# clancylian/retinaface

Hardware: NVIDIA B200
Metric: faces/sec (end-to-end detect) (higher is better)
Workload: dtype f16

## Files before the change

### retinaface_b200/csrc/engine_internal.cuh

```cuda
#pragma once
#include <algorithm>
#include <cstdarg>
#include <cstdio>
#include <cstring>
#include <functional>
#include <map>
#include <memory>
#include <string>
#include <type_traits>
#include <vector>

#include "common.cuh"
#include "host_copy.h"
#include "model.h"
#include "postproc.cuh"
#include "preprocess.cuh"

using namespace rf;

#define RF_STR2(x) #x
#define RF_STR(x) RF_STR2(x)

namespace rf_eng {

struct TileChain;
std::string &create_error();

struct CudaFail { cudaError_t e; const char *what; const char *file; int line; };
struct PlanFail { int status; std::string msg; };
#define CK(call)                                                        \
    do {                                                                \
        cudaError_t _e = (call);                                        \
        if (_e != cudaSuccess) throw CudaFail{_e, #call, __FILE__, __LINE__}; \
    } while (0)

inline std::string fmt(const char *f, ...) {
    char buf[1024];
    va_list ap;
    va_start(ap, f);
    vsnprintf(buf, sizeof buf, f, ap);
    va_end(ap);
    return buf;
}
// ... 179 lines not shown
        size_t off = h->wstage_q.size();
        h->wstage_q.insert(h->wstage_q.end(), v.begin(), v.end());
        while (h->wstage_q.size() % 128) h->wstage_q.push_back(0);
        return off;
    }
    int tensor(const std::string &name, int hh, int ww, int c) {
        TensorInfo t;
        t.name = name; t.h = hh; t.w = ww; t.c = c;
        t.bytes_per_img = (size_t)hh * ww * c * h->elem;
        h->tensors.push_back(t);
        h->tensor_by_name[name] = (int)h->tensors.size() - 1;
        return (int)h->tensors.size() - 1;
    }
    void step(Step s) { h->steps.push_back(std::move(s)); }
};

constexpr int TC_SMEM_LIMIT = 200 * 1024;
struct DwGeom { int rows, nsplit, Rmax; };
template <typename T>
void build_plan(rf_handle h);
cudaError_t tc_init();
std::vector<__half> make_stem_blob(const std::vector<float> &w0, const std::vector<float> &b0, const std::vector<float> &wd,
                                   const std::vector<float> &bd, const std::vector<float> &wp, const std::vector<float> &bp);
int plan_stem_tc(Builder &B);
int plan_pair_legacy(Builder &B, int i, int tin, int ih, int iw);
void plan_conv_legacy(Builder &B, const std::string &sname, std::vector<const FoldedConv *> cs, int tin, int ih, int iw, int t0, int ld0,
                      int off0, int n0, int relu0, int t1, int ld1, int off1, int relu1, int lane = 0, int tup = -1, int up_which = 0);
int plan_fpn_merge_h2(Builder &B, const std::string &name, int tlat, int tup, int fh, int fw, int which);
template <typename T>
void plan_heads_and_nms(Builder &B, bool with_heads, bool with_nms);
std::vector<__half> pack_tc_weights(const std::vector<const FoldedConv *> &cs, std::vector<float> &bias, int &Kpad, int nsplit = 1);
void build_plan_tiles(rf_handle h);
cudaError_t tile_init();
std::string describe_chains(rf_handle h);
void comm_release(rf_handle h);
void comm_wait_in_graph(rf_handle h, int n, cudaStream_t s);
int jpeg_info(rf_handle h, const uint8_t *data, size_t len, int *w, int *hgt);
int jpeg_decode(rf_handle h, const uint8_t *const *data, const size_t *len, int n, uint8_t *const *dst, const int *w, const int *hgt, cudaStream_t s);
void jpeg_release(rf_handle h);
const char *jpeg_backend(rf_handle h);
void build_plan_i8(rf_handle h);
cudaError_t tc_init_i8();

}
```

### retinaface_b200/csrc/plan_fp.cu

```cuda
#include "engine_internal.cuh"
#include "kernels_simt.cuh"
#include "stem_tc.cuh"
#include "tc_conv.cuh"
#include "tc_dwpw2d.cuh"

namespace rf_eng {

#define CK_L(...) CK(launch_k(__VA_ARGS__))

std::vector<float> pack_gemm(const std::vector<const FoldedConv *> &cs, std::vector<float> &bias) {
    const int cin = cs[0]->cin, k = cs[0]->k;
    int N = 0;
    for (auto c : cs) N += c->cout;
    std::vector<float> w((size_t)k * k * cin * N);
    bias.assign(N, 0.f);
    int n0 = 0;
    for (auto c : cs) {
        for (int o = 0; o < c->cout; o++) {
            bias[n0 + o] = c->b[o];
            for (int ci = 0; ci < cin; ci++)
                for (int t = 0; t < k * k; t++)
                    w[((size_t)t * cin + ci) * N + n0 + o] = c->w[((size_t)o * cin + ci) * k * k + t];
        }
        n0 += c->cout;
// ... 56 lines not shown
    TcDwArgs a = a_in;
    a.mul_Wp = fast_div_mul((uint32_t)a.Wp); a.mul_Hp = fast_div_mul((uint32_t)a.Hp);
    a.mul_OW = fast_div_mul((uint32_t)a.OW); a.mul_OH = fast_div_mul((uint32_t)a.OH);
    const long M = (long)a.nimg * a.OH * a.OW;
    dim3 grid((unsigned)((M + a.rows - 1) / a.rows), nsplit);
    const size_t smem = tc_dw_smem_bytes(a);
    switch (tc_tmem_cols(a.N)) {
        case 32: if (a.C >= 64) CK_L(k_tc_dwpw_staged<32, true>, grid, dim3(TC_THREADS), smem, s, a); else CK_L(k_tc_dwpw_staged<32, false>, grid, dim3(TC_THREADS), smem, s, a); break;
        case 64: if (a.C >= 64) CK_L(k_tc_dwpw_staged<64, true>, grid, dim3(TC_THREADS), smem, s, a); else CK_L(k_tc_dwpw_staged<64, false>, grid, dim3(TC_THREADS), smem, s, a); break;
        case 128: if (a.C >= 64) CK_L(k_tc_dwpw_staged<128, true>, grid, dim3(TC_THREADS), smem, s, a); else CK_L(k_tc_dwpw_staged<128, false>, grid, dim3(TC_THREADS), smem, s, a); break;
        default: if (a.C >= 64) CK_L(k_tc_dwpw_staged<256, true>, grid, dim3(TC_THREADS), smem, s, a); else CK_L(k_tc_dwpw_staged<256, false>, grid, dim3(TC_THREADS), smem, s, a); break;
    }
}
void launch_tc_dwpw_2d(const TcDw2dArgs &a, cudaStream_t s) {
    const dim3 grid((unsigned)(a.tiles_x * a.tiles_y * a.nimg));
    const size_t smem = tc_dw2d_smem_bytes(a);
    switch (tc_tmem_cols(a.N)) {
        case 32: CK_L(k_tc_dwpw_2d<32>, grid, dim3(TC_THREADS), smem, s, a); break;
        case 64: CK_L(k_tc_dwpw_2d<64>, grid, dim3(TC_THREADS), smem, s, a); break;
        case 128: CK_L(k_tc_dwpw_2d<128>, grid, dim3(TC_THREADS), smem, s, a); break;
        default: CK_L(k_tc_dwpw_2d<256>, grid, dim3(TC_THREADS), smem, s, a); break;
    }
}

cudaError_t tc_init() {
    cudaError_t e;
#define RF_TC_ATTR(K_) if ((e = cudaFuncSetAttribute(K_, cudaFuncAttributeMaxDynamicSharedMemorySize, TC_SMEM_LIMIT))) return e
    RF_TC_ATTR((k_tc_conv_staged<32, false>)); RF_TC_ATTR((k_tc_conv_staged<64, false>)); RF_TC_ATTR((k_tc_conv_staged<128, false>)); RF_TC_ATTR((k_tc_conv_staged<256, false>));
    RF_TC_ATTR((k_tc_conv_staged<32, true>)); RF_TC_ATTR((k_tc_conv_staged<64, true>)); RF_TC_ATTR((k_tc_conv_staged<128, true>)); RF_TC_ATTR((k_tc_conv_staged<256, true>));
    RF_TC_ATTR((k_tc_dwpw_staged<32, true>)); RF_TC_ATTR((k_tc_dwpw_staged<64, true>)); RF_TC_ATTR((k_tc_dwpw_staged<128, true>)); RF_TC_ATTR((k_tc_dwpw_staged<256, true>));
    RF_TC_ATTR((k_tc_dwpw_staged<32, false>)); RF_TC_ATTR((k_tc_dwpw_staged<64, false>)); RF_TC_ATTR((k_tc_dwpw_staged<128, false>)); RF_TC_ATTR((k_tc_dwpw_staged<256, false>));
    RF_TC_ATTR(k_tc_dwpw_2d<32>); RF_TC_ATTR(k_tc_dwpw_2d<64>); RF_TC_ATTR(k_tc_dwpw_2d<128>); RF_TC_ATTR(k_tc_dwpw_2d<256>);
#undef RF_TC_ATTR
    return cudaSuccess;
}

DwGeom dw_geometry(int C, int N, int IH, int IW, int S) {
    const int OH = IH / S, OW = IW / S, Wp = IW + 2, Hp = IH + 1, Kpad = (C + 15) / 16 * 16;
    auto centre = [&](long m) { long ox = m % OW, oy = (m / OW) % OH, b = m / ((long)OW * OH); return (b * Hp + oy * S) * Wp + ox * S + 1; };
    for (int rows : {128, 64}) {
        if (rows == 128 && OH * OW <= 28 * 28) continue;
        for (int nsplit : {1, 2, 4}) {
            if ((N / nsplit) % 16) continue;
            long g = rows, t = (long)OH * OW;
            while (t) { long u = g % t; g = t; t = u; }
            const long M = ((long)rows / g + 1) * OH * OW;
            int R = 0;
            for (long m0 = 0; m0 < M; m0 += rows) {
                long ml = std::min(m0 + rows, M) - 1;
                R = std::max(R, (int)(centre(ml) - centre(m0) + 2 * (Wp + 1) + 1));
            }
            R |= 1;
            TcDwArgs a{};
            a.C = C; a.Rmax = R; a.Kpad = Kpad; a.N = N / nsplit; a.rows = rows;
            if (R <= TC_MAX_R && tc_dw_smem_bytes(a) <= (size_t)TC_SMEM_LIMIT) return {rows, nsplit, R};
        }
    }
    return {0, 0, 0};
}

std::vector<__half> make_stem_blob(const std::vector<float> &w0, const std::vector<float> &b0, const std::vector<float> &wd,
                                          const std::vector<float> &bd, const std::vector<float> &wp, const std::vector<float> &bp) {
    std::vector<__half> b0img(2 * 4 * 16 * 8, __float2half(0.f)), b1img(2 * 16 * 8, __float2half(0.f));
    for (int k = 0; k < 27; k++)
        for (int o = 0; o < 8; o++) {
            const float wv = w0[k * 8 + o];
            const __half hi = __float2half(wv);
            b0img[((k / 8) * 16 + o) * 8 + (k % 8)] = hi;
            b0img[((4 + k / 8) * 16 + o) * 8 + (k % 8)] = __float2half(wv - __half2float(hi));
        }
    for (int c = 0; c < 8; c++)
        for (int o = 0; o < 16; o++) b1img[(0 * 16 + o) * 8 + c] = __float2half(wp[c * 16 + o]);
    std::vector<__half> blob(STEM_CONST_BYTES / 2, __float2half(0.f));
    memcpy(blob.data(), b0img.data(), STEM_B0_BYTES);
    memcpy(reinterpret_cast<unsigned char *>(blob.data()) + STEM_B0_BYTES, b1img.data(), STEM_B1_BYTES);
    std::vector<float> fl;
    fl.insert(fl.end(), b0.begin(), b0.begin() + 8);
    fl.insert(fl.end(), wd.begin(), wd.begin() + 72);
    fl.insert(fl.end(), bd.begin(), bd.begin() + 8);
    fl.insert(fl.end(), bp.begin(), bp.begin() + 16);
    fl.insert(fl.end(), wp.begin(), wp.begin() + 128);
    memcpy(reinterpret_cast<unsigned char *>(blob.data()) + STEM_B0_BYTES + STEM_B1_BYTES, fl.data(), STEM_F_FLOATS * 4);
    return blob;
}


int plan_pair_legacy(Builder &B, int i, int tin, int ih, int iw) {
    rf_handle h = B.h;
    const Model &m = h->model;
    auto T_ = [h](int id) { return reinterpret_cast<__half *>(h->tptr(id)); };
    auto Wd = [h](size_t off) { return h->d_weights + off; };
    const double es = h->elem;
    const FoldedConv &dw = m.conv("mobilenet0_conv" + std::to_string(i) + "_fwd");
    const FoldedConv &pw = m.conv("mobilenet0_conv" + std::to_string(i + 1) + "_fwd");
    const int C = dw.cout, S = dw.stride;
    std::vector<float> wd(9 * C);
    for (int c = 0; c < C; c++)
        for (int t = 0; t < 9; t++) wd[t * C + c] = dw.w[(size_t)c * 9 + t];
    size_t owd = B.add_weights(wd), obd = B.add_weights(dw.b);
    const int oh = ih / S, ow_ = iw / S;
    const int N = pw.cout;
    const DwGeom geo = dw_geometry(C, N, ih, iw, S);
    if (geo.rows == 0) throw PlanFail{RF_ERR_UNSUPPORTED, fmt("layer mobilenet0_conv%d (%dx%d, %d channels) does not fit shared memory", i, iw, ih, C)};
    std::vector<float> bias;
    int Kpad = 0;
    std::vector<__half> img = pack_tc_weights({&pw}, bias, Kpad, geo.nsplit);
    size_t oimg = B.add_weights_h(img), obp = B.add_weights(bias);
    int tpw = B.tensor("mobilenet0_relu" + std::to_string(i + 1) + "_fwd", oh, ow_, N);
    Step s;
    s.name = fmt("tc_dw%d+pw%d_s%d_%dto%d", i, i + 1, S, C, N);
    s.in = {tin}; s.out = {tpw};
    s.flops_per_img = 2.0 * oh * ow_ * C * 9 + 2.0 * oh * ow_ * C * N;
    s.bytes_per_img = ((double)ih * iw * C + (double)oh * ow_ * N) * es;
    const bool tiles2d = oh * ow_ > 56 * 56 && C >= 16 && C <= 64 && geo.nsplit == 1 && !(h->cfg.flags & RF_FLAG_DW_1D);
    if (tiles2d) s.name = fmt("tc2d_dw%d+pw%d_s%d_%dto%d", i, i + 1, S, C, N);
    s.launch = [=](int n, cudaStream_t st) {
        if (tiles2d) {
            TcDw2dArgs a{};
            a.in = T_(tin); a.C = C; a.nimg = n; a.IH = ih; a.IW = iw; a.OH = oh; a.OW = ow_; a.S = S; a.N = N;
            a.TH = 8;
            const int t16 = (ow_ + 15) / 16, t14 = (ow_ + 13) / 14;
            a.TW = t14 < t16 ? 14 : 16;
            tc_dw2d_finish(a);
            a.wimg = h->d_weights_h + oimg; a.bias = Wd(obp); a.dw_w = Wd(owd); a.dw_b = Wd(obd); a.out = T_(tpw);
            launch_tc_dwpw_2d(a, st);
            return;
        }
        TcDwArgs a{};
        a.in = T_(tin); a.C = C; a.nimg = n; a.IH = ih; a.IW = iw; a.OH = oh; a.OW = ow_; a.S = S;
        a.N = N / geo.nsplit; a.Ntotal = N; a.Kpad = Kpad; a.rows = geo.rows; a.Wp = iw + 2; a.Hp = ih + 1; a.Rmax = geo.Rmax;
        a.wimg = h->d_weights_h + oimg; a.bias = Wd(obp); a.dw_w = Wd(owd); a.dw_b = Wd(obd); a.out = T_(tpw);
        launch_tc_dwpw(a, geo.nsplit, st);
    };
    B.step(std::move(s));
    return tpw;
}

void plan_conv_legacy(Builder &B, const std::string &sname, std::vector<const FoldedConv *> cs, int tin, int ih, int iw, int t0, int ld0,
                      int off0, int n0, int relu0, int t1, int ld1, int off1, int relu1, int lane, int tup, int up_which) {
    rf_handle h = B.h;
    const Model &m = h->model;
    auto T_ = [h](int id) { return reinterpret_cast<__half *>(h->tptr(id)); };
    auto Wd = [h](size_t off) { return h->d_weights + off; };
    const double es = h->elem;
    std::vector<float> bias;
    int Kpad = 0;
    std::vector<__half> img = pack_tc_weights(cs, bias, Kpad);
    size_t oimg = B.add_weights_h(img), ob = B.add_weights(bias);
    const int N = (int)bias.size(), cin = cs[0]->cin, ks = cs[0]->k;
    size_t oup = tup >= 0 ? B.add_weights(m.up_w[up_which]) : 0;
    if (cin & (cin - 1)) throw PlanFail{RF_ERR_UNSUPPORTED, fmt("convolution %s: %d input channels (the tensor-core kernels index by shifts: powers of two only)", sname.c_str(), cin)};
    TcConvArgs probe{};
    probe.Cin = cin; probe.taps = ks * ks; probe.N = N; probe.R = (ks == 3 ? 128 + 2 * (iw + 3) : 128) | 1;
    if (tup >= 0) { probe.up = reinterpret_cast<const __half *>(1); probe.Cmax = (((probe.R / (iw + 2) + 2) / 2 + 3) * (iw / 2)) | 1; }
    if (tc_conv_smem_bytes(probe) > (size_t)TC_SMEM_LIMIT || probe.R > TC_MAX_R)
        throw PlanFail{RF_ERR_UNSUPPORTED, fmt("convolution %s (%dx%d map) does not fit shared memory", sname.c_str(), iw, ih)};
    Step s;
// ... 353 lines not shown
```

### retinaface_b200/csrc/plan_tile.cu

```cuda
#include <cstdlib>

#include "engine_internal.cuh"
#include "tile_chain.cuh"

namespace rf_eng {

namespace {

typedef CUresult (*EncodeTiledFn)(CUtensorMap *, CUtensorMapDataType, cuuint32_t, void *, const cuuint64_t *, const cuuint64_t *,
                                  const cuuint32_t *, const cuuint32_t *, CUtensorMapInterleave, CUtensorMapSwizzle, CUtensorMapL2promotion,
                                  CUtensorMapFloatOOBfill);
EncodeTiledFn g_encode = nullptr;

constexpr int TCH_SMEM_LIMIT = 226 * 1024;

CUtensorMap make_map(const void *base, int C, int W, int H, int n, int bc, int bw, int bh, int es) {
    CUtensorMap m;
    cuuint64_t dims[4] = {(cuuint64_t)C, (cuuint64_t)W, (cuuint64_t)H, (cuuint64_t)n};
    cuuint64_t strides[3] = {(cuuint64_t)C * 2, (cuuint64_t)W * C * 2, (cuuint64_t)H * W * C * 2};
    cuuint32_t box[4] = {(cuuint32_t)bc, (cuuint32_t)bw, (cuuint32_t)bh, 1};
    cuuint32_t est[4] = {1, (cuuint32_t)es, (cuuint32_t)es, 1};
    const CUtensorMapSwizzle sw = bc * 2 == 128 ? CU_TENSOR_MAP_SWIZZLE_128B : (bc * 2 == 64 ? CU_TENSOR_MAP_SWIZZLE_64B : CU_TENSOR_MAP_SWIZZLE_32B);
    CUresult r = g_encode(&m, CU_TENSOR_MAP_DATA_TYPE_FLOAT16, 4, const_cast<void *>(base), dims, strides, box, est, CU_TENSOR_MAP_INTERLEAVE_NONE, sw,
                          CU_TENSOR_MAP_L2_PROMOTION_L2_128B, CU_TENSOR_MAP_FLOAT_OOB_FILL_NONE);
    if (r != CUDA_SUCCESS) throw PlanFail{RF_ERR_CUDA, fmt("cuTensorMapEncodeTiled failed (%d) for a %dx%dx%d tensor, box %dx%dx%d", (int)r, C, W, H, bc, bw, bh)};
    return m;
}

int round_up(int v, int a) { return (v + a - 1) / a * a; }

}

struct TileChain {
    struct LBuf {
        int C = 0;
        int halo = 0;
        bool stored = false;
        int store_tensor = -1;
        int first = 1 << 30, last = -1;
        bool is_input = false, is_merge = false;
    };
    struct LStage {
        int type = TCH_CONV, Cin = 0, N = 0, taps = 1, stride = 1, in_buf = 0;
        std::vector<int> ob_buf, ob_c16, ob_relu;
        std::vector<__half> wd_img, wp_img;
        std::vector<float> bd, bp;
        int hs = 0;
        int store_buf = -1;
        double flops = 0;
    };
    std::string name;
    std::vector<LBuf> bufs;
    std::vector<LStage> stages;
    int in_tensor = -1, in_C = 0, in_W = 0, in_H = 0, in_s2 = 0;
    int W = 0, H = 0;
    int merge_tensor = -1;
    std::vector<__half> merge_w;
    int level = -1;
    bool fused_nms = false;
    TchArgs args{};
    size_t bias_off = 0;
    int store_buf_of[3] = {-1, -1, -1}, store_C[3] = {0, 0, 0};
    int nstores = 0;
// ... 333 lines not shown
void add_chain_step(Builder &B, std::shared_ptr<TileChain> c, int lane, double bytes_per_img) {
    rf_handle h = B.h;
    commit_chain(B, *c);
    h->chains.push_back(c);
    Step s;
    s.name = c->name;
    s.lane = lane;
    s.in = {c->in_tensor};
    if (c->merge_tensor >= 0) s.in.push_back(c->merge_tensor);
    for (int i = 0; i < c->nstores; i++) s.out.push_back(c->bufs[c->store_buf_of[i]].store_tensor);
    double fl = 0;
    for (auto &ls : c->stages) fl += ls.flops * c->W * c->H;
    s.flops_per_img = fl;
    s.bytes_per_img = bytes_per_img;
    s.launch = [h, c](int n, cudaStream_t st) { launch_chain(h, c, n, st); };
    B.step(std::move(s));
}

}

std::string describe_chains(rf_handle h) {
    std::string out;
    for (auto &cp : h->chains) {
        const TileChain &c = *cp;
        const TchArgs &a = c.args;
        out += fmt("%s: %dx%d map, TH=%d HT=%d Wl=%d, %d tiles/image, %d stages, %d MMA tiles/tile, smem %d B (%s weights), TMEM %d x %d cols, stores %d\n",
                   c.name.c_str(), c.W, c.H, a.TH, a.HT, a.Wl, a.tiles_per_img, a.nstages, c.mtiles, a.smem_bytes, a.resident ? "resident" : "streamed", a.nsets,
                   a.set_cols, c.nstores);
    }
    return out;
}

cudaError_t tile_init() {
    if (!g_encode) {
        void *fn = nullptr;
        cudaDriverEntryPointQueryResult q;
        cudaError_t e = cudaGetDriverEntryPoint("cuTensorMapEncodeTiled", &fn, cudaEnableDefault, &q);
        if (e != cudaSuccess) return e;
        if (!fn) return cudaErrorNotSupported;
        g_encode = (EncodeTiledFn)fn;
    }
    return cudaFuncSetAttribute(k_tile_chain<0>, cudaFuncAttributeMaxDynamicSharedMemorySize, TCH_SMEM_LIMIT);
}

enum { TM_A = 1, TM_B = 2, TM_C = 4, TM_D = 8, TM_E = 16, TM_AGGR = 32, TM_SSH = 64, TM_HEAD = 128, TM_NMS = 256, TM_ALL = 511 };
constexpr unsigned TM_LATENCY = TM_SSH | TM_HEAD | TM_NMS;
constexpr unsigned TM_LATENCY_SMALL = TM_AGGR | TM_SSH | TM_HEAD | TM_NMS;
constexpr unsigned TM_THROUGHPUT = 0;

static bool build_tiles_with_mask(rf_handle h, unsigned mask) {
    Builder B{h, h->cfg.net_h, h->cfg.net_w};
    const Model &m = h->model;
    const int H = h->cfg.net_h, W = h->cfg.net_w, mb = h->cfg.max_batch, mf = h->cfg.max_faces;
    if (!(mask & TM_SSH)) mask &= ~(TM_HEAD | TM_NMS);
    if (!(mask & TM_HEAD)) mask &= ~TM_NMS;
    const double es = 2;
    auto pair = [&](int i) -> std::pair<const FoldedConv *, const FoldedConv *> {
        return {&m.conv("mobilenet0_conv" + std::to_string(i) + "_fwd"), &m.conv("mobilenet0_conv" + std::to_string(i + 1) + "_fwd")};
    };
    auto relu_name = [](int i) { return "mobilenet0_relu" + std::to_string(i) + "_fwd"; };

    int cur = plan_stem_tc(B);
    int cur_h = H / 2, cur_w = W / 2, cur_c = 16;

    int lat1 = -1, lat2 = -1, lat3 = -1;
    auto backbone = [&](const std::string &name, std::vector<int> is, bool enabled, const char *lat_conv, int *lat_out, int lane_lat) {
        const int S = pair(is[0]).first->stride;
        const int oh = cur_h / S, ow = cur_w / S;
        const int Cout = pair(is.back()).second->cout;
        bool done = false;
        if (enabled) {
            auto c = std::make_shared<TileChain>();
            c->name = "tile_" + name;
            c->in_tensor = cur; c->in_C = cur_c; c->in_W = cur_w; c->in_H = cur_h; c->in_s2 = S == 2;
// ... 184 lines not shown
```

### retinaface_b200/csrc/tc_conv.cuh

```cuda
#pragma once
#include "common.cuh"

namespace rf {

constexpr int TC_LBO_A = 128 * 16 + 16;

struct TcOut {
    __half *p0; int ld0; int n0; int relu0;
    __half *p1; int ld1; int relu1;
};

namespace tc {

__device__ __forceinline__ uint32_t smem_u32(const void *p) { return (uint32_t)__cvta_generic_to_shared(p); }

__device__ __forceinline__ void mbar_init(uint64_t *bar, unsigned count) {
    asm volatile("mbarrier.init.shared::cta.b64 [%0], %1;" ::"r"(smem_u32(bar)), "r"(count));
}
__device__ __forceinline__ void mbar_expect_tx(uint64_t *bar, unsigned bytes) {
    asm volatile("mbarrier.arrive.expect_tx.shared::cta.b64 _, [%0], %1;" ::"r"(smem_u32(bar)), "r"(bytes) : "memory");
}
__device__ __forceinline__ void mbar_wait(uint64_t *bar, unsigned parity) {
    unsigned done = 0;
    unsigned spins = 0;
    while (!done) {
        asm volatile(
            "{\n\t.reg .pred p;\n\t"
            "mbarrier.try_wait.parity.shared::cta.b64 p, [%1], %2;\n\t"
            "selp.u32 %0, 1, 0, p;\n\t}"
            : "=r"(done)
            : "r"(smem_u32(bar)), "r"(parity)
            : "memory");
        if (!done && ++spins > (1u << 24)) __trap();
    }
}
__device__ __forceinline__ void bulk_g2s(void *dst, const void *src, unsigned bytes, uint64_t *bar) {
    asm volatile("cp.async.bulk.shared::cluster.global.mbarrier::complete_tx::bytes [%0], [%1], %2, [%3];" ::"r"(smem_u32(dst)),
                 "l"(src), "r"(bytes), "r"(smem_u32(bar))
                 : "memory");
}
__device__ __forceinline__ void fence_async_smem() { asm volatile("fence.proxy.async.shared::cta;" ::: "memory"); }
__device__ __forceinline__ void tc_fence_before() { asm volatile("tcgen05.fence::before_thread_sync;" ::: "memory"); }
__device__ __forceinline__ void tc_fence_after() { asm volatile("tcgen05.fence::after_thread_sync;" ::: "memory"); }

template <int COLS>
__device__ __forceinline__ void tmem_alloc(uint32_t *slot) {
    asm volatile("tcgen05.alloc.cta_group::1.sync.aligned.shared::cta.b32 [%0], %1;" ::"r"(smem_u32(slot)), "n"(COLS) : "memory");
    asm volatile("tcgen05.relinquish_alloc_permit.cta_group::1.sync.aligned;" ::: "memory");
}
template <int COLS>
__device__ __forceinline__ void tmem_dealloc(uint32_t addr) {
    asm volatile("tcgen05.dealloc.cta_group::1.sync.aligned.b32 %0, %1;" ::"r"(addr), "n"(COLS) : "memory");
}
__device__ __forceinline__ void mma_commit(uint64_t *bar) {
    asm volatile("tcgen05.commit.cta_group::1.mbarrier::arrive::one.shared::cluster.b64 [%0];" ::"r"(smem_u32(bar)) : "memory");
}
__device__ __forceinline__ void mma_f16(uint32_t d_tmem, uint64_t adesc, uint64_t bdesc, uint32_t idesc, uint32_t accumulate) {
    asm volatile(
        "{\n\t.reg .pred p;\n\t"
        "setp.ne.b32 p, %4, 0;\n\t"
        "tcgen05.mma.cta_group::1.kind::f16 [%0], %1, %2, %3, p;\n\t}"
        ::"r"(d_tmem), "l"(adesc), "l"(bdesc), "r"(idesc), "r"(accumulate)
        : "memory");
}
__device__ __forceinline__ uint64_t smem_desc(uint32_t addr, uint32_t lbo_bytes, uint32_t sbo_bytes) {
    uint64_t d = 0;
    d |= (uint64_t)((addr >> 4) & 0x3FFF);
    d |= (uint64_t)((lbo_bytes >> 4) & 0x3FFF) << 16;
    d |= (uint64_t)((sbo_bytes >> 4) & 0x3FFF) << 32;
    d |= (uint64_t)1 << 46;
    return d;
// ... 424 lines not shown
```

### retinaface_b200/csrc/tc_dwpw2d.cuh

```cuda
#pragma once
#include "tc_conv.cuh"

namespace rf {

struct TcDw2dArgs {
    const __half *in;
    int C, nimg, IH, IW, OH, OW, S;
    int N;
    int TH, TW;
    int tiles_x, tiles_y;
    int PH, PW;
    uint32_t lbo_a;
    uint32_t mul_TW, mul_tiles_x, mul_tiles;
    const __half *wimg;
    const float *bias;
    const float *dw_w, *dw_b;
    __half *out;
};

inline void tc_dw2d_finish(TcDw2dArgs &a) {
    const int G = a.C >> 3;
    a.PH = (a.TH - 1) * a.S + 3;
    a.PW = (a.TW - 1) * a.S + 3;
    a.tiles_x = (a.OW + a.TW - 1) / a.TW;
    a.tiles_y = (a.OH + a.TH - 1) / a.TH;
    a.lbo_a = (uint32_t)(128 + 8 / G) * 16;
    a.mul_TW = fast_div_mul((uint32_t)a.TW);
    a.mul_tiles_x = fast_div_mul((uint32_t)a.tiles_x);
    a.mul_tiles = fast_div_mul((uint32_t)(a.tiles_x * a.tiles_y));
}
inline size_t tc_dw2d_smem_bytes(const TcDw2dArgs &a) {
    return (size_t)a.PH * a.PW * a.C * 2 + (size_t)(a.C / 8) * a.lbo_a + (size_t)a.C * a.N * 2 + 128;
}

#ifndef RF_DW2D_OCC
#define RF_DW2D_OCC 6
#endif
template <int NT>
__global__ void __launch_bounds__(TC_THREADS, RF_DW2D_OCC) k_tc_dwpw_2d(const TcDw2dArgs a) {
    extern __shared__ __align__(128) unsigned char smem[];
    __shared__ __align__(8) uint64_t bar_b, bar_done;
    __shared__ uint32_t s_tmem;
    __shared__ float s_bias[256];
    __shared__ __align__(16) __half s_dwh[9 * 64];
    __shared__ __align__(16) float s_dwb[64];

    const int tid = threadIdx.x, warp = tid >> 5, lane = tid & 31;
    const int G = a.C >> 3, lg = 31 - __clz(G);
    const int PH = a.PH, PW = a.PW;
    const uint32_t lbo_a = a.lbo_a;
    const int pix = a.C * 2;
    unsigned char *sS = smem;
    unsigned char *sA = smem + (size_t)PH * PW * pix;
    unsigned char *sB = sA + (size_t)G * lbo_a;
    const int tiles = a.tiles_x * a.tiles_y;
    const int b = fast_div((int)blockIdx.x, a.mul_tiles), trem = blockIdx.x - b * tiles;
    const int ty0 = fast_div(trem, a.mul_tiles_x);
    const int oy0 = ty0 * a.TH, ox0 = (trem - ty0 * a.tiles_x) * a.TW;
    const int iy0 = oy0 * a.S - 1, ix0 = ox0 * a.S - 1;

    if (tid == 0) {
        tc::mbar_init(&bar_b, 1);
        tc::mbar_init(&bar_done, 1);
        asm volatile("fence.mbarrier_init.release.cluster;" ::: "memory");
        const unsigned bytes = (unsigned)((size_t)a.C * a.N * 2);
        tc::mbar_expect_tx(&bar_b, bytes);
        tc::bulk_g2s(sB, a.wimg, bytes, &bar_b);
    }
    if (warp == 1) tc::tmem_alloc<NT>(&s_tmem);
    pdl_trigger();
    if (tid < a.N) s_bias[tid] = a.bias[tid];
    for (int i = tid; i < 9 * a.C; i += TC_THREADS) s_dwh[i] = __float2half_rn(a.dw_w[i]);
    if (tid < a.C) s_dwb[tid] = a.dw_b[tid];
    pdl_wait();
    {
        const int per_row = PW << lg;
        const int px_lo = max(0, -ix0), px_hi = min(PW, a.IW - ix0);
        const unsigned px_n = (unsigned)max(px_hi - px_lo, 0);
        const uint32_t sS_s = tc::smem_u32(sS);
        for (int py = warp; py < PH; py += TC_THREADS / 32) {
            const int iy = iy0 + py;
            const bool rowok = iy >= 0 && iy < a.IH;
            const __half *src_row = a.in + (ptrdiff_t)(((b * a.IH + (rowok ? iy : 0)) * a.IW + ix0) * a.C);
            const uint32_t dst_row = sS_s + (uint32_t)(py * PW * pix);
            const __half *zsrc = a.in;
            for (int i = lane; i < per_row; i += 32) {
                const bool ok = rowok && (unsigned)((i >> lg) - px_lo) < px_n;
                cp_async16_zfill_s(dst_row + (uint32_t)i * 16u, ok ? src_row + i * 8 : zsrc, ok);
            }
        }
    }
    cp_async_wait_all();
    __syncthreads();
    const int rows = a.TH * a.TW;
    if (a.S == 1) {
        const int items = (a.TH >> 1) * a.TW << lg;
        for (int it = tid; it < items; it += TC_THREADS) {
            const int g = it & (G - 1), rest = it >> lg;
            const int typ = fast_div(rest, a.mul_TW), tx = rest - typ * a.TW;
            const int ty = typ * 2;
            float acc0[8], acc1[8];
            {
                const float4 b0 = *reinterpret_cast<const float4 *>(&s_dwb[g * 8]), b1 = *reinterpret_cast<const float4 *>(&s_dwb[g * 8 + 4]);
                acc0[0] = b0.x; acc0[1] = b0.y; acc0[2] = b0.z; acc0[3] = b0.w; acc0[4] = b1.x; acc0[5] = b1.y; acc0[6] = b1.z; acc0[7] = b1.w;
#pragma unroll
                for (int i = 0; i < 8; i++) acc1[i] = acc0[i];
            }
            const unsigned char *base = sS + (ty * PW + tx) * pix + g * 16;
#pragma unroll 1
            for (int ry = 0; ry < 4; ry++) {
#pragma unroll
                for (int kx = 0; kx < 3; kx++) {
                    const uint4 x = *reinterpret_cast<const uint4 *>(base + (ry * PW + kx) * pix);
                    if (ry < 3) fhfma8(acc0, x, *reinterpret_cast<const uint4 *>(&s_dwh[(ry * 3 + kx) * a.C + g * 8]));
                    if (ry > 0) fhfma8(acc1, x, *reinterpret_cast<const uint4 *>(&s_dwh[((ry - 1) * 3 + kx) * a.C + g * 8]));
                }
            }
#pragma unroll
            for (int i = 0; i < 8; i++) { acc0[i] = fmaxf(acc0[i], 0.f); acc1[i] = fmaxf(acc1[i], 0.f); }
            Vec8<__half> o0, o1;
            o0.from_float(acc0);
            o1.from_float(acc1);
            const int r = ty * a.TW + tx;
            *reinterpret_cast<uint4 *>(sA + (size_t)g * lbo_a + (size_t)r * 16) = o0.v;
            *reinterpret_cast<uint4 *>(sA + (size_t)g * lbo_a + (size_t)(r + a.TW) * 16) = o1.v;
        }
    } else {
        const int items = rows << lg;
        for (int it = tid; it < items; it += TC_THREADS) {
            const int g = it & (G - 1), r = it >> lg;
            const int ty = fast_div(r, a.mul_TW), tx = r - ty * a.TW;
            float acc[8];
            {
                const float4 b0 = *reinterpret_cast<const float4 *>(&s_dwb[g * 8]), b1 = *reinterpret_cast<const float4 *>(&s_dwb[g * 8 + 4]);
                acc[0] = b0.x; acc[1] = b0.y; acc[2] = b0.z; acc[3] = b0.w; acc[4] = b1.x; acc[5] = b1.y; acc[6] = b1.z; acc[7] = b1.w;
            }
            const unsigned char *base = sS + (ty * a.S * PW + tx * a.S) * pix + g * 16;
#pragma unroll
            for (int t = 0; t < 9; t++) {
                fhfma8(acc, *reinterpret_cast<const uint4 *>(base + ((t / 3) * PW + (t % 3)) * pix), *reinterpret_cast<const uint4 *>(&s_dwh[t * a.C + g * 8]));
            }
#pragma unroll
            for (int i = 0; i < 8; i++) acc[i] = fmaxf(acc[i], 0.f);
            Vec8<__half> o;
            o.from_float(acc);
            *reinterpret_cast<uint4 *>(sA + (size_t)g * lbo_a + (size_t)r * 16) = o.v;
        }
    }
    tc::fence_async_smem();
    tc::tc_fence_before();
    __syncthreads();
    tc::tc_fence_after();
    const uint32_t tmem = s_tmem;
    if (tid == 0) {
        tc::mbar_wait(&bar_b, 0);
        tc::tc_fence_after();
        const uint32_t idesc = (1u << 4) | ((uint32_t)(a.N >> 3) << 17) | ((uint32_t)(128 >> 4) << 24);
        const uint32_t a_addr = tc::smem_u32(sA), b_addr = tc::smem_u32(sB);
        const uint32_t lbo_b = (uint32_t)a.N * 16;
        for (int ks = 0; ks < (a.C >> 4); ks++) {
            const uint64_t ad = tc::smem_desc(a_addr + (uint32_t)(2 * ks) * lbo_a, lbo_a, 128);
            const uint64_t bd = tc::smem_desc(b_addr + (uint32_t)(2 * ks) * lbo_b, lbo_b, 128);
            tc::mma_f16(tmem, ad, bd, idesc, ks > 0 ? 1u : 0u);
        }
        tc::mma_commit(&bar_done);
    }
    if (warp == 0) tc::mbar_wait(&bar_done, 0);
    __syncthreads();
    tc::tc_fence_after();
    {
        const int r = (warp & 3) * 32 + lane;
        const int ty = fast_div(r, a.mul_TW), tx = r - ty * a.TW;
        const int oy = oy0 + ty, ox = ox0 + tx;
        const bool ok = r < rows && oy < a.OH && ox < a.OW;
        TcOut o{a.out, a.N, a.N, 1, nullptr, 0, 0};
        tc_epilogue(tmem, a.N, s_bias, o, ok ? (long)((b * a.OH + oy) * a.OW + ox) : -1, 0);
    }
    tc::tc_fence_before();
    __syncthreads();
    if (warp == 1) tc::tmem_dealloc<NT>(tmem);
}

}
```

### retinaface_b200/csrc/tile_chain.cuh

```cuda
#pragma once
#include <cuda.h>

#include "common.cuh"
#include "postproc_dev.cuh"
#include "tc_conv.cuh"

namespace rf {

constexpr int TCH_THREADS = 320;
constexpr int TCH_MAX_STAGES = 8;
constexpr int TCH_MAX_BUFS = 8;
constexpr int TCH_EPI_THREADS = 256;
enum { TCH_CONV = 0, TCH_DWPW = 1, TCH_HEAD = 2 };

struct TchBuf {
    int off;
    int row;
    int slabs;
    int slab_stride;
    int rows_lo;
    int nrows;
    int slack;
};

// ... 21 lines not shown
    int nms_smem;
    float *blobs[3];
};

struct TchArgs {
    int nstages, nbufs;
    TchStage st[TCH_MAX_STAGES];
    TchBuf buf[TCH_MAX_BUFS];
    int Wl, HT, TH;
    int W, H, nimg, tiles_per_img, ntiles;
    int nsets, set_cols;
    int wd_smem, wp_smem, bias_smem, smem_bytes;
    int resident;
    unsigned *dbg;
    unsigned long long *trace;
    const unsigned char *warena;
    const float *bias;
    int bias_floats;
    int in_s2, plane_stride, in_C;
    unsigned in_bytes;
    int merge_C, merge_buf, merge_rows, merge_w_bias;
    unsigned merge_bytes;
    TchHead head;
};

struct TchMaps {
    CUtensorMap in;
    CUtensorMap aux;
    CUtensorMap st[3];
};

namespace tch {

__device__ __forceinline__ void tma_load_4d(uint32_t dst, const CUtensorMap *map, uint64_t *bar, int c0, int c1, int c2, int c3) {
    asm volatile("cp.async.bulk.tensor.4d.shared::cluster.global.mbarrier::complete_tx::bytes [%0], [%1, {%3, %4, %5, %6}], [%2];"
                 ::"r"(dst), "l"(map), "r"(tc::smem_u32(bar)), "r"(c0), "r"(c1), "r"(c2), "r"(c3)
                 : "memory");
}
__device__ __forceinline__ void tma_store_4d(const CUtensorMap *map, uint32_t src, int c0, int c1, int c2, int c3) {
    asm volatile("cp.async.bulk.tensor.4d.global.shared::cta.bulk_group [%0, {%2, %3, %4, %5}], [%1];"
                 ::"l"(map), "r"(src), "r"(c0), "r"(c1), "r"(c2), "r"(c3)
                 : "memory");
}
__device__ __forceinline__ void wait(uint64_t *bar, unsigned parity, unsigned *dbg, unsigned code) {
    unsigned done = 0, spins = 0;
    while (!done) {
        asm volatile(
            "{\n\t.reg .pred p;\n\t"
            "mbarrier.try_wait.parity.shared::cta.b64 p, [%1], %2;\n\t"
            "selp.u32 %0, 1, 0, p;\n\t}"
            : "=r"(done)
            : "r"(tc::smem_u32(bar)), "r"(parity)
            : "memory");
        if (!done && ++spins > (1u << 22)) {
            if (dbg) { *reinterpret_cast<volatile unsigned *>(dbg) = code | (blockIdx.x << 20); __threadfence_system(); __nanosleep(2000000); }
            __trap();
        }
    }
}
__device__ __forceinline__ void wait_warp(uint64_t *bar, unsigned parity, unsigned *dbg, unsigned code) {
    wait(bar, parity, dbg, code);
    __syncwarp();
}
#ifdef RF_TCH_TRACE
__device__ __forceinline__ void trace(unsigned long long *t, unsigned code) {
    if (t && blockIdx.x == 0) {
        unsigned long long now;
        asm volatile("mov.u64 %0, %%globaltimer;" : "=l"(now));
        const unsigned i = atomicAdd(reinterpret_cast<unsigned *>(t), 1u);
        if (i < 500) { t[1 + 2 * i] = code; t[2 + 2 * i] = now; }
    }
// ... 606 lines not shown
```

Baseline: 478,300.

## Load 2D dw+pw input halo via TMA tensor map and bulk-copy packed constants

The 2D depthwise+pointwise tensor-core kernel now fetches its padded input halo tile with a single 4D TMA tensor load, which zero-fills out-of-bounds elements, in place of per-thread cp.async with zfill. The pointwise weights, fp16 depthwise weights and both biases are packed at plan time into one blob and brought into shared memory with bulk async copies, removing the per-block float-to-half conversion and scalar loads. A tensor map is encoded on the host at each launch and passed as a grid constant. The shared buffer is realigned to 128 bytes. This aims to cut address arithmetic and load-issue overhead in the prologue, at the cost of host-side map encoding per launch.

```diff
diff --git a/retinaface_b200/csrc/engine_internal.cuh b/retinaface_b200/csrc/engine_internal.cuh
--- a/retinaface_b200/csrc/engine_internal.cuh
+++ b/retinaface_b200/csrc/engine_internal.cuh
@@ -9,6 +9,8 @@
 #include <string>
 #include <type_traits>
 #include <vector>
+
+#include <cuda.h>
 
 #include "common.cuh"
 #include "host_copy.h"
@@ -254,6 +256,8 @@
 std::vector<__half> pack_tc_weights(const std::vector<const FoldedConv *> &cs, std::vector<float> &bias, int &Kpad, int nsplit = 1);
 void build_plan_tiles(rf_handle h);
 cudaError_t tile_init();
+cudaError_t map_encoder_init();
+CUtensorMap make_map(const void *base, int C, int W, int H, int n, int bc, int bw, int bh, int es, bool swizzle = true);
 std::string describe_chains(rf_handle h);
 void comm_release(rf_handle h);
 void comm_wait_in_graph(rf_handle h, int n, cudaStream_t s);
diff --git a/retinaface_b200/csrc/plan_fp.cu b/retinaface_b200/csrc/plan_fp.cu
--- a/retinaface_b200/csrc/plan_fp.cu
+++ b/retinaface_b200/csrc/plan_fp.cu
@@ -112,7 +112,7 @@
     RF_TC_ATTR((k_tc_dwpw_staged<32, false>)); RF_TC_ATTR((k_tc_dwpw_staged<64, false>)); RF_TC_ATTR((k_tc_dwpw_staged<128, false>)); RF_TC_ATTR((k_tc_dwpw_staged<256, false>));
     RF_TC_ATTR(k_tc_dwpw_2d<32>); RF_TC_ATTR(k_tc_dwpw_2d<64>); RF_TC_ATTR(k_tc_dwpw_2d<128>); RF_TC_ATTR(k_tc_dwpw_2d<256>);
 #undef RF_TC_ATTR
-    return cudaSuccess;
+    return map_encoder_init();
 }
 
 DwGeom dw_geometry(int C, int N, int IH, int IW, int S) {
@@ -177,32 +177,38 @@
     std::vector<float> wd(9 * C);
     for (int c = 0; c < C; c++)
         for (int t = 0; t < 9; t++) wd[t * C + c] = dw.w[(size_t)c * 9 + t];
-    size_t owd = B.add_weights(wd), obd = B.add_weights(dw.b);
     const int oh = ih / S, ow_ = iw / S;
     const int N = pw.cout;
     const DwGeom geo = dw_geometry(C, N, ih, iw, S);
     if (geo.rows == 0) throw PlanFail{RF_ERR_UNSUPPORTED, fmt("layer mobilenet0_conv%d (%dx%d, %d channels) does not fit shared memory", i, iw, ih, C)};
+    const bool tiles2d = oh * ow_ > 56 * 56 && C >= 16 && C <= 64 && geo.nsplit == 1 && !(h->cfg.flags & RF_FLAG_DW_1D);
     std::vector<float> bias;
     int Kpad = 0;
     std::vector<__half> img = pack_tc_weights({&pw}, bias, Kpad, geo.nsplit);
-    size_t oimg = B.add_weights_h(img), obp = B.add_weights(bias);
+    size_t oimg = 0, owd = 0, obd = 0, obp = 0;
+    if (tiles2d) {
+        oimg = B.add_weights_h(tc_dw2d_pack(img, wd, dw.b, bias));
+    } else {
+        oimg = B.add_weights_h(img); obp = B.add_weights(bias);
+        owd = B.add_weights(wd); obd = B.add_weights(dw.b);
+    }
     int tpw = B.tensor("mobilenet0_relu" + std::to_string(i + 1) + "_fwd", oh, ow_, N);
     Step s;
     s.name = fmt("tc_dw%d+pw%d_s%d_%dto%d", i, i + 1, S, C, N);
     s.in = {tin}; s.out = {tpw};
     s.flops_per_img = 2.0 * oh * ow_ * C * 9 + 2.0 * oh * ow_ * C * N;
     s.bytes_per_img = ((double)ih * iw * C + (double)oh * ow_ * N) * es;
-    const bool tiles2d = oh * ow_ > 56 * 56 && C >= 16 && C <= 64 && geo.nsplit == 1 && !(h->cfg.flags & RF_FLAG_DW_1D);
     if (tiles2d) s.name = fmt("tc2d_dw%d+pw%d_s%d_%dto%d", i, i + 1, S, C, N);
     s.launch = [=](int n, cudaStream_t st) {
         if (tiles2d) {
             TcDw2dArgs a{};
-            a.in = T_(tin); a.C = C; a.nimg = n; a.IH = ih; a.IW = iw; a.OH = oh; a.OW = ow_; a.S = S; a.N = N;
+            a.C = C; a.nimg = n; a.IH = ih; a.IW = iw; a.OH = oh; a.OW = ow_; a.S = S; a.N = N;
             a.TH = 8;
             const int t16 = (ow_ + 15) / 16, t14 = (ow_ + 13) / 14;
             a.TW = t14 < t16 ? 14 : 16;
             tc_dw2d_finish(a);
-            a.wimg = h->d_weights_h + oimg; a.bias = Wd(obp); a.dw_w = Wd(owd); a.dw_b = Wd(obd); a.out = T_(tpw);
+            a.in = make_map(T_(tin), C, iw, ih, n, C, a.PW, a.PH, 1, false);
+            a.consts = reinterpret_cast<const unsigned char *>(h->d_weights_h + oimg); a.out = T_(tpw);
             launch_tc_dwpw_2d(a, st);
             return;
         }
diff --git a/retinaface_b200/csrc/plan_tile.cu b/retinaface_b200/csrc/plan_tile.cu
--- a/retinaface_b200/csrc/plan_tile.cu
+++ b/retinaface_b200/csrc/plan_tile.cu
@@ -6,29 +6,42 @@
 namespace rf_eng {
 
 namespace {
+
+constexpr int TCH_SMEM_LIMIT = 226 * 1024;
+
+int round_up(int v, int a) { return (v + a - 1) / a * a; }
+
+}
 
 typedef CUresult (*EncodeTiledFn)(CUtensorMap *, CUtensorMapDataType, cuuint32_t, void *, const cuuint64_t *, const cuuint64_t *,
                                   const cuuint32_t *, const cuuint32_t *, CUtensorMapInterleave, CUtensorMapSwizzle, CUtensorMapL2promotion,
                                   CUtensorMapFloatOOBfill);
-EncodeTiledFn g_encode = nullptr;
-
-constexpr int TCH_SMEM_LIMIT = 226 * 1024;
-
-CUtensorMap make_map(const void *base, int C, int W, int H, int n, int bc, int bw, int bh, int es) {
+static EncodeTiledFn g_encode = nullptr;
+
+cudaError_t map_encoder_init() {
+    if (!g_encode) {
+        void *fn = nullptr;
+        cudaDriverEntryPointQueryResult q;
+        cudaError_t e = cudaGetDriverEntryPoint("cuTensorMapEncodeTiled", &fn, cudaEnableDefault, &q);
+        if (e != cudaSuccess) return e;
+        if (!fn) return cudaErrorNotSupported;
+        g_encode = (EncodeTiledFn)fn;
+    }
+    return cudaSuccess;
+}
+
+CUtensorMap make_map(const void *base, int C, int W, int H, int n, int bc, int bw, int bh, int es, bool swizzle) {
     CUtensorMap m;
     cuuint64_t dims[4] = {(cuuint64_t)C, (cuuint64_t)W, (cuuint64_t)H, (cuuint64_t)n};
     cuuint64_t strides[3] = {(cuuint64_t)C * 2, (cuuint64_t)W * C * 2, (cuuint64_t)H * W * C * 2};
     cuuint32_t box[4] = {(cuuint32_t)bc, (cuuint32_t)bw, (cuuint32_t)bh, 1};
     cuuint32_t est[4] = {1, (cuuint32_t)es, (cuuint32_t)es, 1};
-    const CUtensorMapSwizzle sw = bc * 2 == 128 ? CU_TENSOR_MAP_SWIZZLE_128B : (bc * 2 == 64 ? CU_TENSOR_MAP_SWIZZLE_64B : CU_TENSOR_MAP_SWIZZLE_32B);
+    const CUtensorMapSwizzle sw = !swizzle ? CU_TENSOR_MAP_SWIZZLE_NONE
+                                  : bc * 2 == 128 ? CU_TENSOR_MAP_SWIZZLE_128B : (bc * 2 == 64 ? CU_TENSOR_MAP_SWIZZLE_64B : CU_TENSOR_MAP_SWIZZLE_32B);
     CUresult r = g_encode(&m, CU_TENSOR_MAP_DATA_TYPE_FLOAT16, 4, const_cast<void *>(base), dims, strides, box, est, CU_TENSOR_MAP_INTERLEAVE_NONE, sw,
                           CU_TENSOR_MAP_L2_PROMOTION_L2_128B, CU_TENSOR_MAP_FLOAT_OOB_FILL_NONE);
     if (r != CUDA_SUCCESS) throw PlanFail{RF_ERR_CUDA, fmt("cuTensorMapEncodeTiled failed (%d) for a %dx%dx%d tensor, box %dx%dx%d", (int)r, C, W, H, bc, bw, bh)};
     return m;
-}
-
-int round_up(int v, int a) { return (v + a - 1) / a * a; }
-
 }
 
 struct TileChain {
@@ -428,14 +441,8 @@
 }
 
 cudaError_t tile_init() {
-    if (!g_encode) {
-        void *fn = nullptr;
-        cudaDriverEntryPointQueryResult q;
-        cudaError_t e = cudaGetDriverEntryPoint("cuTensorMapEncodeTiled", &fn, cudaEnableDefault, &q);
-        if (e != cudaSuccess) return e;
-        if (!fn) return cudaErrorNotSupported;
-        g_encode = (EncodeTiledFn)fn;
-    }
+    cudaError_t e = map_encoder_init();
+    if (e != cudaSuccess) return e;
     return cudaFuncSetAttribute(k_tile_chain<0>, cudaFuncAttributeMaxDynamicSharedMemorySize, TCH_SMEM_LIMIT);
 }
 
diff --git a/retinaface_b200/csrc/tc_conv.cuh b/retinaface_b200/csrc/tc_conv.cuh
--- a/retinaface_b200/csrc/tc_conv.cuh
+++ b/retinaface_b200/csrc/tc_conv.cuh
@@ -1,4 +1,6 @@
 #pragma once
+#include <cuda.h>
+
 #include "common.cuh"
 
 namespace rf {
@@ -37,6 +39,11 @@
 __device__ __forceinline__ void bulk_g2s(void *dst, const void *src, unsigned bytes, uint64_t *bar) {
     asm volatile("cp.async.bulk.shared::cluster.global.mbarrier::complete_tx::bytes [%0], [%1], %2, [%3];" ::"r"(smem_u32(dst)),
                  "l"(src), "r"(bytes), "r"(smem_u32(bar))
+                 : "memory");
+}
+__device__ __forceinline__ void tma_load_4d(uint32_t dst, const CUtensorMap *map, uint64_t *bar, int c0, int c1, int c2, int c3) {
+    asm volatile("cp.async.bulk.tensor.4d.shared::cluster.global.mbarrier::complete_tx::bytes [%0], [%1, {%3, %4, %5, %6}], [%2];"
+                 ::"r"(dst), "l"(map), "r"(smem_u32(bar)), "r"(c0), "r"(c1), "r"(c2), "r"(c3)
                  : "memory");
 }
 __device__ __forceinline__ void fence_async_smem() { asm volatile("fence.proxy.async.shared::cta;" ::: "memory"); }
diff --git a/retinaface_b200/csrc/tc_dwpw2d.cuh b/retinaface_b200/csrc/tc_dwpw2d.cuh
--- a/retinaface_b200/csrc/tc_dwpw2d.cuh
+++ b/retinaface_b200/csrc/tc_dwpw2d.cuh
@@ -1,10 +1,13 @@
 #pragma once
+#include <cstring>
+#include <vector>
+
 #include "tc_conv.cuh"
 
 namespace rf {
 
 struct TcDw2dArgs {
-    const __half *in;
+    CUtensorMap in;
     int C, nimg, IH, IW, OH, OW, S;
     int N;
     int TH, TW;
@@ -12,9 +15,7 @@
     int PH, PW;
     uint32_t lbo_a;
     uint32_t mul_TW, mul_tiles_x, mul_tiles;
-    const __half *wimg;
-    const float *bias;
-    const float *dw_w, *dw_b;
+    const unsigned char *consts;
     __half *out;
 };
 
@@ -29,6 +30,20 @@
     a.mul_tiles_x = fast_div_mul((uint32_t)a.tiles_x);
     a.mul_tiles = fast_div_mul((uint32_t)(a.tiles_x * a.tiles_y));
 }
+__host__ __device__ __forceinline__ size_t tc_dw2d_const_bytes(int C, int N) { return (size_t)C * N * 2 + (size_t)9 * C * 2 + (size_t)C * 4 + (size_t)N * 4; }
+inline std::vector<__half> tc_dw2d_pack(const std::vector<__half> &bimg, const std::vector<float> &wd, const std::vector<float> &bd,
+                                        const std::vector<float> &bias) {
+    const int C = (int)bd.size(), N = (int)bias.size();
+    std::vector<__half> blob(tc_dw2d_const_bytes(C, N) / 2);
+    unsigned char *p = reinterpret_cast<unsigned char *>(blob.data());
+    memcpy(p, bimg.data(), (size_t)C * N * 2);
+    p += (size_t)C * N * 2;
+    for (int i = 0; i < 9 * C; i++) reinterpret_cast<__half *>(p)[i] = __float2half_rn(wd[i]);
+    p += (size_t)9 * C * 2;
+    memcpy(p, bd.data(), (size_t)C * 4);
+    memcpy(p + (size_t)C * 4, bias.data(), (size_t)N * 4);
+    return blob;
+}
 inline size_t tc_dw2d_smem_bytes(const TcDw2dArgs &a) {
     return (size_t)a.PH * a.PW * a.C * 2 + (size_t)(a.C / 8) * a.lbo_a + (size_t)a.C * a.N * 2 + 128;
 }
@@ -37,11 +52,11 @@
 #define RF_DW2D_OCC 6
 #endif
 template <int NT>
-__global__ void __launch_bounds__(TC_THREADS, RF_DW2D_OCC) k_tc_dwpw_2d(const TcDw2dArgs a) {
+__global__ void __launch_bounds__(TC_THREADS, RF_DW2D_OCC) k_tc_dwpw_2d(const __grid_constant__ TcDw2dArgs a) {
     extern __shared__ __align__(128) unsigned char smem[];
-    __shared__ __align__(8) uint64_t bar_b, bar_done;
+    __shared__ __align__(8) uint64_t bar_b, bar_in, bar_done;
     __shared__ uint32_t s_tmem;
-    __shared__ float s_bias[256];
+    __shared__ __align__(16) float s_bias[256];
     __shared__ __align__(16) __half s_dwh[9 * 64];
     __shared__ __align__(16) float s_dwb[64];
 
@@ -50,8 +65,8 @@
     const int PH = a.PH, PW = a.PW;
     const uint32_t lbo_a = a.lbo_a;
     const int pix = a.C * 2;
-    unsigned char *sS = smem;
-    unsigned char *sA = smem + (size_t)PH * PW * pix;
+    unsigned char *sS = smem + ((128u - (tc::smem_u32(smem) & 127u)) & 127u);
+    unsigned char *sA = sS + (size_t)PH * PW * pix;
     unsigned char *sB = sA + (size_t)G * lbo_a;
     const int tiles = a.tiles_x * a.tiles_y;
     const int b = fast_div((int)blockIdx.x, a.mul_tiles), trem = blockIdx.x - b * tiles;
@@ -61,36 +76,28 @@
 
     if (tid == 0) {
         tc::mbar_init(&bar_b, 1);
+        tc::mbar_init(&bar_in, 1);
         tc::mbar_init(&bar_done, 1);
         asm volatile("fence.mbarrier_init.release.cluster;" ::: "memory");
-        const unsigned bytes = (unsigned)((size_t)a.C * a.N * 2);
-        tc::mbar_expect_tx(&bar_b, bytes);
-        tc::bulk_g2s(sB, a.wimg, bytes, &bar_b);
+        const unsigned bw = (unsigned)(a.C * a.N * 2), bd = (unsigned)(9 * a.C * 2);
+        tc::mbar_expect_tx(&bar_b, (unsigned)tc_dw2d_const_bytes(a.C, a.N));
+        tc::bulk_g2s(sB, a.consts, bw, &bar_b);
+        tc::bulk_g2s(s_dwh, a.consts + bw, bd, &bar_b);
+        tc::bulk_g2s(s_dwb, a.consts + bw + bd, (unsigned)a.C * 4, &bar_b);
+        tc::bulk_g2s(s_bias, a.consts + bw + bd + a.C * 4, (unsigned)a.N * 4, &bar_b);
     }
     if (warp == 1) tc::tmem_alloc<NT>(&s_tmem);
     pdl_trigger();
-    if (tid < a.N) s_bias[tid] = a.bias[tid];
-    for (int i = tid; i < 9 * a.C; i += TC_THREADS) s_dwh[i] = __float2half_rn(a.dw_w[i]);
-    if (tid < a.C) s_dwb[tid] = a.dw_b[tid];
     pdl_wait();
-    {
-        const int per_row = PW << lg;
-        const int px_lo = max(0, -ix0), px_hi = min(PW, a.IW - ix0);
-        const unsigned px_n = (unsigned)max(px_hi - px_lo, 0);
-        const uint32_t sS_s = tc::smem_u32(sS);
-        for (int py = warp; py < PH; py += TC_THREADS / 32) {
-            const int iy = iy0 + py;
-            const bool rowok = iy >= 0 && iy < a.IH;
-            const __half *src_row = a.in + (ptrdiff_t)(((b * a.IH + (rowok ? iy : 0)) * a.IW + ix0) * a.C);
-            const uint32_t dst_row = sS_s + (uint32_t)(py * PW * pix);
-            const __half *zsrc = a.in;
-            for (int i = lane; i < per_row; i += 32) {
-                const bool ok = rowok && (unsigned)((i >> lg) - px_lo) < px_n;
-                cp_async16_zfill_s(dst_row + (uint32_t)i * 16u, ok ? src_row + i * 8 : zsrc, ok);
-            }
-        }
+    if (tid == 0) {
+        tc::mbar_expect_tx(&bar_in, (unsigned)(PH * PW * pix));
+        tc::tma_load_4d(tc::smem_u32(sS), &a.in, &bar_in, 0, ix0, iy0, b);
     }
-    cp_async_wait_all();
+    if (warp == 0) {
+        __syncwarp();
+        tc::mbar_wait(&bar_b, 0);
+        tc::mbar_wait(&bar_in, 0);
+    }
     __syncthreads();
     const int rows = a.TH * a.TW;
     if (a.S == 1) {
@@ -153,8 +160,6 @@
     tc::tc_fence_after();
     const uint32_t tmem = s_tmem;
     if (tid == 0) {
-        tc::mbar_wait(&bar_b, 0);
-        tc::tc_fence_after();
         const uint32_t idesc = (1u << 4) | ((uint32_t)(a.N >> 3) << 17) | ((uint32_t)(128 >> 4) << 24);
         const uint32_t a_addr = tc::smem_u32(sA), b_addr = tc::smem_u32(sB);
         const uint32_t lbo_b = (uint32_t)a.N * 16;
diff --git a/retinaface_b200/csrc/tile_chain.cuh b/retinaface_b200/csrc/tile_chain.cuh
--- a/retinaface_b200/csrc/tile_chain.cuh
+++ b/retinaface_b200/csrc/tile_chain.cuh
@@ -77,11 +77,7 @@
 
 namespace tch {
 
-__device__ __forceinline__ void tma_load_4d(uint32_t dst, const CUtensorMap *map, uint64_t *bar, int c0, int c1, int c2, int c3) {
-    asm volatile("cp.async.bulk.tensor.4d.shared::cluster.global.mbarrier::complete_tx::bytes [%0], [%1, {%3, %4, %5, %6}], [%2];"
-                 ::"r"(dst), "l"(map), "r"(tc::smem_u32(bar)), "r"(c0), "r"(c1), "r"(c2), "r"(c3)
-                 : "memory");
-}
+using tc::tma_load_4d;
 __device__ __forceinline__ void tma_store_4d(const CUtensorMap *map, uint32_t src, int c0, int c1, int c2, int c3) {
     asm volatile("cp.async.bulk.tensor.4d.global.shared::cta.bulk_group [%0, {%2, %3, %4, %5}], [%1];"
                  ::"l"(map), "r"(src), "r"(c0), "r"(c1), "r"(c2), "r"(c3)
```

Result: faster. 488,600 (median of 6 runs) (+2.1%).
